# roboyu/Kimera-Multi

Hardware: AMD Instinct MI355X
Metric: dpgo edges*iters/sec (+ LC candidates verified/sec in 'lcd') (higher is better)
Workload: dtype f64

## Files before the change

### kimera-multi_amd/csrc/pgo.hip

```cpp
#include <hip/hip_runtime.h>
#include <hip/hip_ext.h>
#include <rccl/rccl.h>
#include <dlfcn.h>

#include <algorithm>
#include <chrono>
#include <thread>
#include <type_traits>
#include <cmath>
#include <cstdio>
#include <cstdlib>
#include <cstring>
#include <limits>
#include <numeric>
#include <string>
#include <vector>

#include "common.h"

#ifndef KMX_HESS_PROBE
#define KMX_HESS_PROBE 0
#endif

namespace {
// ... 1168 lines not shown
    for (int k = 0; k < j; ++k) s -= Lm[j * 4 + k] * Lm[j * 4 + k];
    Lm[j * 4 + j] = sqrt(s);
    for (int ii = j + 1; ii < 4; ++ii) {
      double t = A[ii * 4 + j];
      for (int k = 0; k < j; ++k) t -= Lm[ii * 4 + k] * Lm[j * 4 + k];
      Lm[ii * 4 + j] = t / Lm[j * 4 + j];
    }
  }
  for (int c = 0; c < 4; ++c)
    for (int ii = 0; ii < 4; ++ii) {
      double s = (ii == c) ? 1.0 : 0.0;
      for (int k = c; k < ii; ++k) s -= Lm[ii * 4 + k] * Li[k * 4 + c];
      Li[ii * 4 + c] = (ii < c) ? 0.0 : s / Lm[ii * 4 + ii];
    }
  double* Pi = d.Pinv + SYM4 * (size_t)pose;
  int j = 0;
  for (int x = 0; x < 4; ++x)
    for (int y = x; y < 4; ++y) {
      double s = 0.0;
      for (int k = 0; k < 4; ++k) s += Li[k * 4 + x] * Li[k * 4 + y];
      Pi[j++] = s;
    }
}

template <int R, int RW, int RM>
__device__ __forceinline__ void body_grad(const Dev& d, int gated, char* smem) {
  const Lane L = lane_map<R>(d);
  if (gated) {
    if (L.tile == 0 && threadIdx.x == 0) store_gnc(d.gnc, load_gnc(d.gnc_next));
    if (d.gnc_next->fired) {
      const int np = L.np, p0 = L.p0;
      for (int t = threadIdx.x; t < np; t += blockDim.x) pose_precond<RW>(d, p0 + t);
      __syncthreads();
    }
  }
  if (d.ctl[L.l].phase != PH_START) return;
  double y[4] = {0, 0, 0, 0}, G[4], cost = 0.0;
  hinc_grad<R, RW>(d, L, d.X, d.pub, G, &cost, smem);
  if (L.valid) load4(d.X + (size_t)L.pose * 4 * R + 4 * L.a, y);
  constexpr int NDP = R >= 5 ? 1 : 2;
  double2 dpart[NDP];
  {
    const double2* Dp2 = reinterpret_cast<const double2*>(d.hD + SYM4 * (size_t)L.pose);
#pragma unroll
    for (int u = 0; u < NDP; ++u) {
      const int i = L.a + u * R;
      dpart[u] = (L.valid && i < 5) ? Dp2[i] : make_double2(0.0, 0.0);
    }
  }
  double S[9], gr[4], zr[4];
  double* scr = reinterpret_cast<double*>(smem);
  group_symYtG<R, true>(y, G, L.base, S, scr);
#pragma unroll
  for (int c = 0; c < 3; ++c) gr[c] = G[c] - (y[0] * S[0 * 3 + c] + y[1] * S[1 * 3 + c] + y[2] * S[2 * 3 + c]);
  gr[3] = G[3];
  group_precon<R, true>(d, L.pose, L.valid, y, gr, L.base, zr, scr);
  double vals[3] = {cost, 0.0, 0.0};
  if (L.valid) {
    vals[1] = gr[0] * gr[0] + gr[1] * gr[1] + gr[2] * gr[2] + gr[3] * gr[3];
    vals[2] = zr[0] * gr[0] + zr[1] * gr[1] + zr[2] * gr[2] + zr[3] * gr[3];
  }
  finish_tile<RED_GRAD, 3, RM>(d, L, vals, smem + SmemHG<R>::red_off, [&]() {
    if (!L.valid) return;
    const size_t o = (size_t)L.pose * 4 * R + 4 * L.a;
    store4(d.g + o, gr);
    store4(d.z + o, zr);
    if (L.a == 0) {
      double* Sp = d.S + 6 * (size_t)L.pose;
      Sp[0] = S[0]; Sp[1] = S[1]; Sp[2] = S[2]; Sp[3] = S[4]; Sp[4] = S[5]; Sp[5] = S[8];
    }
    double2* Fp2 = reinterpret_cast<double2*>(d.hDS + SYM4 * (size_t)L.pose);
#pragma unroll
    for (int u = 0; u < NDP; ++u) {
      const int i = L.a + u * R;
      if (i < 5) {
        const double sx = i == 0 ? S[0] : i == 1 ? S[2] : i == 2 ? S[4] : 0.0;
        const double sy = i == 0 ? S[1] : i == 2 ? S[5] : i == 3 ? S[8] : 0.0;
        Fp2[i] = make_double2(dpart[u].x - sx, dpart[u].y - sy);
      }
    }
  });
}

template <bool LAST>
__device__ __forceinline__ void eta_rows(const Dev& d, int l, size_t o, int T, double clast, double et[4]) {
  const int dhn = d.dhn;
  const int F = T > 0 ? (T - 1) / dhn * dhn : 0;
  if (F > 0) load4(d.eta + o, et);
  double dd[DHMAX][4];
#pragma unroll
  for (int i = 0; i < DHMAX; ++i)
    if (F + i < T) load4(d.dh + (size_t)i * d.vec + o, dd[i]);
  const double* ch = d.coefh + (size_t)l * d.p.tcg_max;
#pragma unroll
  for (int i = 0; i < DHMAX; ++i)
    if (F + i < T) {
      const double cj = (LAST && F + i == T - 1) ? clast : ch[F + i];
#pragma unroll
      for (int k = 0; k < 4; ++k) et[k] += cj * dd[i][k];
    }
}

template <int R>
__device__ __forceinline__ void trial_rows(const Dev& d, const Lane& L, size_t o, const double x[4],
                                           const double gg[4], const double rr[4], const double et[4], char* smem) {
  double xt[4];
  group_retract<R>(x, et, L.base, xt);
  double vals[2] = {0.0, 0.0};
  if (L.valid) {
    store4(d.Xt + o, xt);
    double m = 0.0, ch = 0.0;
#pragma unroll
    for (int k = 0; k < 4; ++k) {
      m += et[k] * (gg[k] + rr[k]);
      const double dd = xt[k] - x[k];
      ch += dd * dd;
    }
    vals[0] = m;
    vals[1] = ch;
  }
  double* lds = reinterpret_cast<double*>(smem);
#pragma unroll
  for (int s = 0; s < 2; ++s) {
    const double w = wave_sum(vals[s]);
    if ((threadIdx.x & 63) == 0) lds[s * WAVES + (threadIdx.x >> 6)] = w;
  }
  __syncthreads();
  if (threadIdx.x == 0) {
#pragma unroll
    for (int s = 0; s < 2; ++s) {
      double t = 0.0;
#pragma unroll
      for (int w = 0; w < WAVES; ++w) t += lds[s * WAVES + w];
      d.part[(size_t)L.tile * NPART + 2 + s] = t;
    }
  }
}

template <int R, int RW, int RM>
struct HessPF {
  static constexpr bool rows = RW == 10 && (R >= 5 || RM == RM_CONSUMER);
};
template <int R, int RW, int RM, bool GRAD, bool EARLY>
__device__ __forceinline__ void body_hess(const Dev& d, int gated, int slot, HostStatus* hs,
                                          unsigned long long seq, char* smem) {
  static_assert(RM == RM_CONSUMER || (!GRAD && !EARLY), "the launched form has one body");
  const Lane L = lane_map<R>(d);
  int tcg_iter;
  double beta;
  double y[4] = {0, 0, 0, 0}, zs[4] = {0, 0, 0, 0}, H[4];
  const size_t o = (size_t)L.pose * 4 * R + 4 * L.a;
  const int dhn = d.dhn;
  double dold[4] = {0, 0, 0, 0}, hold[4] = {0, 0, 0, 0};
  double2 dg[5];
  bool first;
  auto epi = [&]() {
    if (L.valid) {
#if KMX_HESS_PROBE & 2
      for (int k = 0; k < 4; ++k) zs[k] = 1e-3 * k;
      for (int c = 0; c < 5; ++c) dg[c] = make_double2(c == 0 || c == 2 ? 1.0 : 0.0, c >= 3 ? 1.0 : 0.0);
#else
      load4(d.z + o, zs);
      const double2* p2 = reinterpret_cast<const double2*>(d.hDS + SYM4 * (size_t)L.pose);
#pragma unroll
      for (int c = 0; c < 5; ++c) dg[c] = p2[c];
#endif
      if (!first) {
        load4(d.dh + (size_t)((tcg_iter - 1) % dhn) * d.vec + o, dold);
        load4(d.hd + o, hold);
      }
    }
  };
  if constexpr (RM == RM_CONSUMER) {
    __shared__ Ctl cs;
    __shared__ double rl[NPART * WAVES];
    const Ctl& c0 = d.ctl[L.l];
    const bool writer = L.tile == L.rt0;
    if (writer && threadIdx.x < (int)(sizeof(Ctl) / 8))
      reinterpret_cast<double*>(&cs)[threadIdx.x] = reinterpret_cast<const double*>(&c0)[threadIdx.x];
    using RS = std::conditional_t<GRAD, RobotSum<3>, RobotSum<2>>;
    const double* const part = GRAD ? d.part : d.part_u;
    constexpr int stride = GRAD ? NPART : 2;
    RS rs;
// ... 25 lines not shown
      if (writer && threadIdx.x == 0) {
        control_on(cs, d, L.l, GRAD ? RED_GRAD : RED_UPDATE, tot, R, true);
        d.ctl2[L.l] = cs;
        if (hs) post_status(hs, L.l, seq, cs.phase == PH_TCG);
      }
      return !u.done;
    };
    bool go;
    if constexpr (EARLY) {
      go = hinc_gather<R, RW, false, false, HessPF<R, RW, RM>::rows>(d, L, d.z, H, smem, decide, epi);
    } else {
      auto epi_late = [&]() {
        epi();
        rs.issue(part, stride, L.rt0, L.rt1);
      };
      hinc_gather<R, RW, false, false, HessPF<R, RW, RM>::rows>(d, L, d.z, H, smem, NoPre{}, epi_late);
      go = decide();
    }
    if (!go) return;
    beta = u.beta;
  } else {
    const Ctl& c = d.ctl[L.l];
    const int ph = c.phase;
    tcg_iter = c.tcg_iter;
    beta = c.beta;
    first = (tcg_iter == 0) || (KMX_HESS_PROBE & 4);
    if (gated && ph != PH_TCG) return;
    if (!hinc_gather<R, RW, true, false, HessPF<R, RW, RM>::rows>(d, L, d.z, H, smem,
                                                                  [&]() { return ph == PH_TCG; }, epi))
      return;
  }
  if (L.valid) {
    double Dg[16];
    expand_sym4(dg, Dg);
#pragma unroll
    for (int c = 0; c < 4; ++c)
      H[c] += zs[0] * Dg[4 * c] + zs[1] * Dg[4 * c + 1] + zs[2] * Dg[4 * c + 2] + zs[3] * Dg[4 * c + 3];
  }
  double hz[4];
#pragma unroll
  for (int k = 0; k < 4; ++k) hz[k] = H[k];
  (void)y;
  double v = 0.0;
  double dl[4] = {0, 0, 0, 0}, hdl[4] = {0, 0, 0, 0};
  if (L.valid) {
    if (first) {
#pragma unroll
      for (int k = 0; k < 4; ++k) { dl[k] = -zs[k]; hdl[k] = -hz[k]; }
    } else {
#pragma unroll
      for (int k = 0; k < 4; ++k) {
        dl[k] = -zs[k] + beta * dold[k];
        hdl[k] = -hz[k] + beta * hold[k];
      }
      if (tcg_iter >= dhn && tcg_iter % dhn == 0) {
        double et[4] = {0, 0, 0, 0};
        if (tcg_iter > dhn) load4(d.eta + o, et);
        const double* ch = d.coefh + (size_t)L.l * d.p.tcg_max;
        for (int j = tcg_iter - dhn; j < tcg_iter; ++j) {
          double dj[4];
          if (j + 1 < tcg_iter) {
            load4(d.dh + (size_t)(j % dhn) * d.vec + o, dj);
          } else {
#pragma unroll
            for (int k = 0; k < 4; ++k) dj[k] = dold[k];
          }
          const double cj = ch[j];
#pragma unroll
          for (int k = 0; k < 4; ++k) et[k] += cj * dj[k];
        }
        store4(d.eta + o, et);
      }
    }
    v = dl[0] * hdl[0] + dl[1] * hdl[1] + dl[2] * hdl[2] + dl[3] * hdl[3];
  }
  finish_tile<RED_HESS, 1, RM>(d, L, &v, smem + SmemH<R>::red_off, [&]() {
    if (L.valid && !(KMX_HESS_PROBE & 8)) {
      store4(d.dh + (size_t)(tcg_iter % dhn) * d.vec + o, dl);
      store4(d.hd + o, hdl);
    }
  });
}

template <int R, int RM>
__device__ __forceinline__ void body_update(const Dev& d, HostStatus* hs, unsigned long long seq, int slot,
                                            char* smem) {
  const Lane L = lane_map<R>(d);
  int tcg_iter, mode;
  double coef;
  const size_t o = (size_t)L.pose * 4 * R + 4 * L.a;
  double rr[4] = {0, 0, 0, 0}, y[4] = {0, 0, 0, 0}, hdl[4] = {0, 0, 0, 0};
  if constexpr (RM == RM_CONSUMER) {
    __shared__ Ctl cs;
    __shared__ double rl[NPART * WAVES];
    Ctl* const cin = d.ctl2;
    Ctl* const cout = d.ctl;
    const Ctl& cq = cin[L.l];
    const bool writer = L.tile == L.rt0;
    if (writer && threadIdx.x < (int)(sizeof(Ctl) / 8))
      reinterpret_cast<double*>(&cs)[threadIdx.x] = reinterpret_cast<const double*>(&cq)[threadIdx.x];
    if (cq.phase != PH_TCG) {
      if (cq.phase == PH_STEP && !cq.retracted) {
        const size_t o2 = (size_t)L.pose * 4 * R + 4 * L.a;
        double x[4] = {0, 0, 0, 0}, gg[4] = {0, 0, 0, 0}, rr2[4] = {0, 0, 0, 0}, et[4] = {0, 0, 0, 0};
        if (L.valid) {
          load4(d.X + o2, x);
          load4(d.g + o2, gg);
          load4(d.r + o2, rr2);
          eta_rows<false>(d, L.l, o2, cq.tcg_iter, 0.0, et);
        }
        trial_rows<R>(d, L, o2, x, gg, rr2, et, smem);
        if (writer) ctl_publish(cout + L.l, cs, true);
        return;
      }
      if (writer) ctl_publish(cout + L.l, cs, false);
      return;
    }
    const bool first0 = cq.tcg_iter == 0;
    RobotSum<1, 4> rs;
    rs.issue(d.part_h, 2, L.rt0, L.rt1);
    if (L.valid) {
      load4(d.hd + o, hdl);
      load4((first0 ? d.g : d.r) + o, rr);
      load4(d.X + o, y);
    }
    double tot[NPART] = {0.0, 0.0, 0.0, 0.0};
    rs.finish(d.part_h, 2, rl, tot);
    const HessStep hsx = hess_step(cq.z_r, cq.e_Pe, cq.e_Pd, cq.d_Pd, cq.Delta, tot[0]);
    if (writer && threadIdx.x < 64) {
      if (threadIdx.x == 0) {
        control_on(cs, d, L.l, RED_HESS, tot, R, true);
        if (slot >= 0) atomicAdd(d.hv_launch + slot, 1);
      }
      __builtin_amdgcn_wave_barrier();
      asm volatile("" ::: "memory");
      ctl_publish(cout + L.l, cs, false);
    }
    tcg_iter = cq.tcg_iter + 1;
    mode = hsx.boundary ? MODE_BOUNDARY : MODE_INTERIOR;
    coef = hsx.coef;
  } else {
    const Ctl& c = d.ctl[L.l];
    if (c.phase != PH_TCG) {
      if (hs && threadIdx.x == 0 && L.tile == L.rt0) post_status(hs, L.l, seq, false);
      return;
    }
    tcg_iter = c.tcg_iter;
    mode = c.mode;
    coef = c.coef;
    if (L.valid) {
      load4(d.hd + o, hdl);
      load4((tcg_iter == 1 ? d.g : d.r) + o, rr);
      load4(d.X + o, y);
    }
  }
  const bool interior = (mode == MODE_INTERIOR);
  (void)tcg_iter;
  {
    double hp[4];
    group_proj<R, true>(y, hdl, L.base, hp, reinterpret_cast<double*>(smem));
    if (L.valid) {
#pragma unroll
      for (int k = 0; k < 4; ++k) rr[k] += coef * hp[k];
    }
  }
  double vals[2] = {0.0, 0.0}, zr[4] = {0, 0, 0, 0};
  if (interior) {
    group_precon<R, true>(d, L.pose, L.valid, y, rr, L.base, zr, reinterpret_cast<double*>(smem));
    if (L.valid) {
      vals[0] = rr[0] * rr[0] + rr[1] * rr[1] + rr[2] * rr[2] + rr[3] * rr[3];
      vals[1] = zr[0] * rr[0] + zr[1] * rr[1] + zr[2] * rr[2] + zr[3] * rr[3];
    }
  }
  finish_tile<RED_UPDATE, 2, RM>(d, L, vals, smem + SmemU::red_off, [&]() {
    if (L.valid) {
      store4(d.r + o, rr);
      if (interior) store4(d.z + o, zr);
    }
  });
}

__device__ __forceinline__ void onesync_scalars(double al, const double* tot, double* rrn, double* zrn) {
#pragma clang fp contract(off)
  *rrn = fmax(tot[2] + 2.0 * al * tot[5] + al * al * tot[6], 0.0);
  *zrn = tot[1] + al * tot[3] + al * al * tot[4];
}

template <int U>
struct RobotSum8 {
  double a[U][8];
  int t0, t1;
  __device__ __forceinline__ void load(const double* part, int tb) {
#pragma unroll
    for (int u = 0; u < U; ++u) {
      const int t = min(tb + (int)threadIdx.x + u * RBLOCK, t1 - 1);
#pragma unroll
      for (int k = 0; k < 4; ++k) {
        const double2 x = ldpart(part, (size_t)t * 8 + 2 * k);
        a[u][2 * k] = x.x;
        a[u][2 * k + 1] = x.y;
      }
    }
  }
  __device__ __forceinline__ void issue(const double* part, int t0_, int t1_) {
    t0 = t0_;
    t1 = t1_;
    if (t1 - t0 <= U * RBLOCK) load(part, t0);
  }
  __device__ __forceinline__ void finish(const double* part, double* lds, double tot[8]) {
    constexpr int RW_ = RBLOCK / 64;
    double v[8];
#pragma unroll
    for (int k = 0; k < 8; ++k) v[k] = 0.0;
    for (int tb = t0; tb < t1; tb += U * RBLOCK) {
      if (t1 - t0 > U * RBLOCK) load(part, tb);
#pragma unroll
      for (int u = 0; u < U; ++u)
        if (tb + (int)threadIdx.x + u * RBLOCK < t1 && threadIdx.x < RBLOCK) {
#pragma unroll
          for (int k = 0; k < 8; ++k) v[k] += a[u][k];
        }
    }
    __syncthreads();
#pragma unroll
    for (int k = 0; k < 8; ++k) {
      const double w = wave_sum(v[k]);
      if ((threadIdx.x & 63) == 0 && threadIdx.x < RBLOCK) lds[k * RW_ + (threadIdx.x >> 6)] = w;
    }
    __syncthreads();
#pragma unroll
    for (int k = 0; k < 8; ++k) {
      double acc = 0.0;
#pragma unroll
      for (int w = 0; w < RW_; ++w) acc += lds[k * RW_ + w];
      tot[k] = acc;
    }
  }
};

template <int R, int W = WAVES>
struct SmemF {
  static constexpr int red_off = SmemH<R, W>::red_off;
  static constexpr int bytes = red_off + 8 * 8 * W + 16;
};

__device__ __forceinline__ double dot4(const double a[4], const double b[4]) {
  return a[0] * b[0] + a[1] * b[1] + a[2] * b[2] + a[3] * b[3];
}

// ... 191 lines not shown
#pragma unroll
  for (int s2 = 0; s2 < 7; ++s2) {
    const double w = wave_sum(pv[s2]);
    if ((threadIdx.x & 63) == 0) lds[s2 * WAVES + (threadIdx.x >> 6)] = w;
  }
  __syncthreads();
  if (threadIdx.x < 8) {
    double t = 0.0;
    if (threadIdx.x < 7) {
#pragma unroll
      for (int w = 0; w < WAVES; ++w) t += lds[threadIdx.x * WAVES + w];
    }
    d.part_f[((size_t)(kn & 1) * d.ntiles + L.tile) * 8 + threadIdx.x] = t;
  }
  if (L.valid) {
    store4(d.dh + (size_t)(kn % dhn) * d.vec + o, dl);
    store4(d.hd + o, hdl);
    store4(d.hz + o, hzn);
    if (!grad) store4(d.z + o, zn);
    store4(((kn & 1) ? d.w1 : d.w0) + o, wn);
    store4(d.r + o, rn);
  }
#ifdef KMX_STEP_STAMPS
  KMX_SS(6);
  if (kn == 2 && threadIdx.x == 0 && L.tile < STEP_STAMP_TILES) {
    for (int i = 0; i < 7; ++i) g_step_stamp[(size_t)L.tile * 16 + i] = ss_[i];
    g_step_stamp[(size_t)L.tile * 16 + 8] = (unsigned long long)L.np;
    g_step_stamp[(size_t)L.tile * 16 + 9] = (unsigned long long)L.n;
    g_step_stamp[(size_t)L.tile * 16 + 10] = (unsigned long long)blockIdx.x;
    g_step_stamp[(size_t)L.tile * 16 + 11] = (unsigned long long)(L.tile == L.rt0);
  }
#endif
}

template <int R>
__device__ __forceinline__ void body_retract(const Dev& d, int fold, const Ctl* src, char* smem) {
  const Lane L = lane_map<R>(d);
  const Ctl& c = src[L.l];
  __shared__ int sph;
  __shared__ double rl[NPART * WAVES];
  if (threadIdx.x == 0) {
    sph = c.phase;
    if (src != d.ctl && L.tile == L.rt0) d.ctl[L.l] = c;
  }
  __syncthreads();
  const int ph = sph;
  const size_t o = (size_t)L.pose * 4 * R + 4 * L.a;
  double x[4] = {0, 0, 0, 0}, et[4] = {0, 0, 0, 0}, gg[4] = {0, 0, 0, 0}, rr[4] = {0, 0, 0, 0}, dl[4];
  if (fold && ph == PH_TCG) {
    RobotSum<2> rs;
    rs.issue(d.part_u, 2, L.rt0, L.rt1);
    double tot[NPART] = {0.0, 0.0, 0.0, 0.0};
    rs.finish(d.part_u, 2, rl, tot);
    const UpdStep u = upd_step(c.mode, c.r_stop, c.lin_stop, c.z_r, c.tcg_iter, tot[0], tot[1], d.p);
    if (!u.done) return;
    if (threadIdx.x == 0 && L.tile == L.rt0) {
      if (u.stop >= 0) d.ctl[L.l].tcg_stop = u.stop;
      d.ctl[L.l].phase = PH_STEP;
    }
  } else if (ph != PH_STEP || (fold == 2 && c.retracted)) {
    return;
  }
  if (L.valid) {
    load4(d.X + o, x);
    load4(d.g + o, gg);
    load4(d.r + o, rr);
    if (d.p.rgd) {
      load4(d.z + o, dl);
      const double coef = c.coef;
#pragma unroll
      for (int k = 0; k < 4; ++k) et[k] += coef * dl[k];
    } else {
      eta_rows<false>(d, L.l, o, c.tcg_iter, 0.0, et);
    }
  }
  trial_rows<R>(d, L, o, x, gg, rr, et, smem);
}

template <int R, int RW, int RM>
__device__ __forceinline__ void body_cost(const Dev& d, const Ctl* src, char* smem) {
  const Lane L = lane_map<R>(d);
  const Ctl& c = src[L.l];
  if (src != d.ctl && threadIdx.x == 0 && L.tile == L.rt0) d.ctl[L.l] = c;
  if (c.phase != PH_STEP) return;
  double cost = inc_owner_cost<R, RW>(d, L, d.Xt, d.pub, smem);
  finish_tile<RED_COST, 1, RM>(d, L, &cost, smem + SmemC<R>::red_off, []() {});
}

template <int R>
__device__ __forceinline__ void body_commit(const Dev& d, int fold, int final) {
  const Lane L = lane_map<R>(d);
  if (final && L.tile == 0 && threadIdx.x == 0) {
    d.gnc->inner += 1;
    d.gnc->rounds += 1;
  }
  bool commit;
  if (fold) {
    __shared__ int sph;
    __shared__ Ctl cs;
    __shared__ double rl[NPART * WAVES];
    const Ctl& c = d.ctl[L.l];
    const bool writer = L.tile == L.rt0;
    if (writer && threadIdx.x < (int)(sizeof(Ctl) / 8))
      reinterpret_cast<double*>(&cs)[threadIdx.x] = reinterpret_cast<const double*>(&c)[threadIdx.x];
    if (threadIdx.x == 0) sph = c.phase;
    __syncthreads();
    if (sph != PH_STEP) return;
    RobotSum<NPART> rs;
    rs.issue(d.part, NPART, L.rt0, L.rt1);
    double tot[NPART] = {0.0, 0.0, 0.0, 0.0};
    rs.finish(d.part, NPART, rl, tot);
    if (d.p.rgd) {
      commit = true;
    } else {
      const double model_dec = -0.5 * tot[2];
      const double rho = (model_dec > 0.0) ? (c.f_cur - tot[0]) / model_dec : -1.0;
      commit = rho > d.p.accept_rho;
    }
    if (threadIdx.x == 0 && writer) {
      control_on(cs, d, L.l, RED_COST, tot, R, true);
      cs.phase = PH_STEP;
      d.ctl[L.l] = cs;
    }
  } else {
    commit = d.ctl[L.l].commit != 0;
  }
  if (!commit || !L.valid) return;
  const size_t o = (size_t)L.pose * 4 * R + 4 * L.a;
  double v[4];
  load4(d.Xt + o, v);
  store4(d.X + o, v);
  if (!final) return;
  const int s = d.pose_slot[L.pose];
  if (s >= 0) store4(d.pub + (size_t)s * 4 * R + 4 * L.a, v);
}

template <int R, int RW, int RM>
__global__ __launch_bounds__(BLOCK, LB<R>::w) void k_grad(Dev d, int gated) {
  KMX_SMEM;
  body_grad<R, RW, RM>(d, gated, smem);
}
template <int R, int RW, int RM, bool GRAD, bool EARLY>
__global__ __launch_bounds__(BLOCK, LB<R>::w) void k_hess(Dev d, int gated, int slot, HostStatus* hs,
                                                          unsigned long long seq) {
  KMX_SMEM;
  body_hess<R, RW, RM, GRAD, EARLY>(d, gated, slot, hs, seq, smem);
}
template <int R, int RM>
__global__ __launch_bounds__(BLOCK) void k_update(Dev d, HostStatus* hs, unsigned long long seq, int slot) {
  KMX_SMEM;
  body_update<R, RM>(d, hs, seq, slot, smem);
}
template <int R, int RW>
__global__ __launch_bounds__(BLOCK, (R <= 5 ? 3 : 2)) void k_step(Dev d, const Ctl* cin, Ctl* cout, int jl, int slot,
                                                                  HostStatus* hs, unsigned long long seq) {
  KMX_SMEM;
  body_step<R, RW>(d, cin, cout, jl, slot, hs, seq, smem);
}
template <int R>
__global__ __launch_bounds__(BLOCK) void k_retract(Dev d, int fold, const Ctl* src) {
  KMX_SMEM;
  body_retract<R>(d, fold, src, smem);
}
template <int R, int RW, int RM>
__global__ __launch_bounds__(BLOCK, LB<R>::w) void k_cost(Dev d, const Ctl* src) {
  KMX_SMEM;
  body_cost<R, RW, RM>(d, src, smem);
}
template <int R>
__global__ __launch_bounds__(BLOCK) void k_commit(Dev d, int fold, int final) {
  body_commit<R>(d, fold, final);
}

__device__ __forceinline__ bool gnc_should_update(const Dev& d) {
  const Params& P = d.p;
  if (!P.robust || !P.gnc_on) return false;
  const Gnc& s = *d.gnc;
  if (s.updates >= P.max_updates) return false;
  if (s.inner > P.inner_iters) return true;
  for (int l = 0; l < d.L; ++l)
    if (!(d.relc[l] <= P.rel_tol)) return false;
  for (int k = 0; k < P.n_ext; ++k)
    if (!(d.ext[k] <= P.rel_tol)) return false;
  return true;
}

template <int RW>
__device__ __forceinline__ void gnc_edge(const Dev& d, int i, int R_, double mu) {
  const int e = d.gnc_edge[i];
  const int2 en = d.gnc_ends[i];
  const int ps = 4 * R_;
  const double* Xi = en.x >= 0 ? d.X + (size_t)en.x * ps : d.pub + (size_t)(-1 - en.x) * ps;
  const double* Xj = en.y >= 0 ? d.X + (size_t)en.y * ps : d.pub + (size_t)(-1 - en.y) * ps;
  const int2 ip = d.eipos[e];
  double2 q[Rec<RW>::Q];
  Rec<RW>::load(d, (size_t)(ip.x >= 0 ? ip.x : ip.y), q);
  Edge E;
  Rec<RW>::edge(q, E);
  double sR = 0.0, sT = 0.0;
  for (int a = 0; a < R_; ++a) {
    const double* yi = Xi + 4 * a;
    const double* yj = Xj + 4 * a;
    for (int c = 0; c < 3; ++c) {
      const double r = yj[c] - (yi[0] * E.R[0 * 3 + c] + yi[1] * E.R[1 * 3 + c] + yi[2] * E.R[2 * 3 + c]);
      sR += r * r;
    }
    const double et = yj[3] - yi[3] - (yi[0] * E.t[0] + yi[1] * E.t[1] + yi[2] * E.t[2]);
    sT += et * et;
  }
  const double rSq = d.ekappa[e] * sR + d.etau[e] * sT;
  const double barcSq = d.p.barc * d.p.barc;
  const double upper = (mu + 1.0) / mu * barcSq;
  const double lower = mu / (mu + 1.0) * barcSq;
  double w;
  if (rSq >= upper) w = 0.0;
  else if (rSq <= lower) w = 1.0;
  else w = sqrt(barcSq * mu * (mu + 1.0) / rSq) - mu;
  d.ew[e] = w;
  const double wk = w * d.ekappa[e], wt = w * d.etau[e];
  constexpr int WK = Rec<RW>::WK;
  constexpr int GS = Rec<RW>::GS;
  if (ip.x >= 0) { d.rec[(size_t)GS * ip.x + WK] = wk; d.rec[(size_t)GS * ip.x + WK + 1] = Rec<RW>::wt_word(wt, true); }
  if (ip.y >= 0) { d.rec[(size_t)GS * ip.y + WK] = wk; d.rec[(size_t)GS * ip.y + WK + 1] = Rec<RW>::wt_word(wt, false); }
}

__device__ __forceinline__ void begin_robot(const Dev& d, const unsigned char* active, int l) {
  Ctl& c = d.ctl[l];
  const bool a = active ? active[l] != 0 : true;
  const Ctl zero = {};
  c = zero;
  c.phase = a ? PH_START : PH_IDLE;
  c.updated = a ? 1 : 0;
  c.Delta = d.p.Delta0;
}

enum BeginMode { BEGIN_ROUND = 1, BEGIN_FORCE_GNC = 2, BEGIN_SOLO = 4 };

template <int RW>
__global__ void k_begin(Dev d, const unsigned char* active, int mode, int R_) {
  const bool fire = d.p.robust && ((mode & BEGIN_FORCE_GNC) ? true : gnc_should_update(d));
  const double mu = d.gnc->mu;
  if (blockIdx.x == 0) {
    if (mode & BEGIN_ROUND)
      for (int l = threadIdx.x; l < d.L; l += blockDim.x) begin_robot(d, active, l);
    if (threadIdx.x == 0) {
      Gnc s = load_gnc(d.gnc);
      s.fired = fire ? 1 : 0;
      if (fire) {
        s.inner = 0;
        s.updates += 1;
        s.mu = mu * d.p.mu_step;
      }
      store_gnc(d.gnc_next, s);
      if (mode & BEGIN_SOLO) store_gnc(d.gnc, s);
// ... 307 lines not shown
  bool own_stream = false;
  int n_robots = 0;
  std::vector<int> npose;
  std::vector<int> local_of;
  std::vector<int> robots;
  std::vector<int> loff;
  int nloc = 0;
  int64_t m_global = 0;
  int64_t npub = 0, first_owned = 0, n_owned = 0;
  std::vector<int64_t> pub_key;
  int mloc = 0;
  std::vector<int64_t> loc_edge_gid;
  int ninc = 0;
  int rw = 10;
  int64_t nshared = 0;
  int n_sh_local = 0, n_gnc = 0, n_osh = 0;
  std::vector<long long> m_robot;
  int ntiles = 0;
  std::vector<int> rt0_h;
  int gnc_on = 0, gnc_inner_iters = 20, gnc_max_updates = 0x7fffffff, n_ext = 0;
  double gnc_rel_tol = 1e-3;
  Dev dv{};
  TileDesc* d_tile = nullptr;
  int* d_rtile0 = nullptr;
  int* d_inc_ptr = nullptr;
  double* d_rec = nullptr;
  int* d_rec_o = nullptr;
  double *d_ekappa = nullptr, *d_etau = nullptr, *d_ew = nullptr;
  int2* d_eipos = nullptr;
  double* d_vec = nullptr;
  double* d_coefh = nullptr;
  double* d_part_f = nullptr;
  int ctl_par = 0;
  double *d_S = nullptr, *d_Pinv = nullptr, *d_hD = nullptr, *d_hDS = nullptr, *d_pub = nullptr, *d_part = nullptr;
  Ctl* d_ctl = nullptr;
  Ctl* d_ctl2 = nullptr;
  double *d_part_h = nullptr, *d_part_u = nullptr;
  Counters* d_cnt = nullptr;
  long long* d_m_robot = nullptr;
  int* d_n_robot = nullptr;
  int* d_pub_src = nullptr;
  int* d_own_src = nullptr;
  int* d_pose_slot = nullptr;
  int* d_gnc_edge = nullptr;
  int2* d_gnc_ends = nullptr;
  int *d_sh_edge = nullptr, *d_sh_idx = nullptr;
  int *d_osh_edge = nullptr, *d_osh_idx = nullptr;
  double* d_relc = nullptr;
  Gnc* d_gnc = nullptr;
  double* d_ext = nullptr;
  int ext_cap = 0;
  unsigned char* d_active = nullptr;
  double* d_scratch = nullptr;
  size_t scratch_cap = 0;
  HostStatus* hstat = nullptr;
  int hstat_cap = 0;
  unsigned long long seq = 0;
  bool poll = true;
  bool poll_auto = true;
  ncclComm_t comm = nullptr;
  int world = 1, rank = 0;
  bool xchg = false, xchg_self_p2p = false;
  int *d_xs_slots = nullptr, *d_xr_slots = nullptr, *d_xs_seg = nullptr, *d_xr_seg = nullptr;
  int *d_xs_rseg = nullptr, *d_xr_rseg = nullptr;
  double *d_xsbuf = nullptr, *d_xrbuf = nullptr;
  long long xn_send = 0, xn_recv = 0;
  std::vector<long long> xs_cnt, xr_cnt, xs_off, xr_off;
  static constexpr int BLIND_SLACK = 2, BLIND_WINDOW = 8;
  static constexpr int MAX_GROUPS = 4;
  struct Group {
    int l0 = 0, l1 = 0;
    int t0 = 0, nt = 0;
    int blind_left = 0;
  };
  int groups_req = 2;
  std::vector<Group> grp;
  Group all;
  int grm = 2;
  int grm_forced = -1;
  static constexpr int GROUP_CONSUMER_MAX_TILES = 384;
  hipStream_t gstream[MAX_GROUPS - 1] = {nullptr, nullptr, nullptr};
  hipEvent_t ev_fork = nullptr, ev_join[MAX_GROUPS - 1] = {nullptr, nullptr, nullptr};
  bool hess_gate = true;
  int rm = RM_LAUNCH;
  int rm_forced = -1;
  int early_stop = 1;
  int decide_forced = -1;
  static constexpr int RM_CONSUMER_MAX_POSES = 80000;
  bool poll_timeout = false;
  bool timing = false;
  int* d_hv_launch = nullptr;
  std::vector<hipEvent_t> ev_pool;
  size_t ev_used = 0;
  double *d_accV = nullptr, *d_accY = nullptr;
  double acc_gamma = 0.0;
  int acc_k = 0;
  bool acc_ready = false, acc_started = false;
};

namespace {

void rot_to_quat(const double* R, double* q) {
  const double tr = R[0] + R[4] + R[8];
  double w, x, y, z;
  if (tr > 0.0) {
    const double s = 2.0 * std::sqrt(tr + 1.0);
    w = 0.25 * s; x = (R[7] - R[5]) / s; y = (R[2] - R[6]) / s; z = (R[3] - R[1]) / s;
  } else if (R[0] > R[4] && R[0] > R[8]) {
    const double s = 2.0 * std::sqrt(1.0 + R[0] - R[4] - R[8]);
    w = (R[7] - R[5]) / s; x = 0.25 * s; y = (R[1] + R[3]) / s; z = (R[2] + R[6]) / s;
  } else if (R[4] > R[8]) {
    const double s = 2.0 * std::sqrt(1.0 + R[4] - R[0] - R[8]);
    w = (R[2] - R[6]) / s; x = (R[1] + R[3]) / s; y = 0.25 * s; z = (R[5] + R[7]) / s;
  } else {
    const double s = 2.0 * std::sqrt(1.0 + R[8] - R[0] - R[4]);
    w = (R[3] - R[1]) / s; x = (R[2] + R[6]) / s; y = (R[5] + R[7]) / s; z = 0.25 * s;
  }
  const double n = std::sqrt(w * w + x * x + y * y + z * z);
  q[0] = w / n; q[1] = x / n; q[2] = y / n; q[3] = z / n;
}
int quat_pack(const double* q, double* q3) {
  int big = 0;
  for (int i = 1; i < 4; ++i)
    if (std::fabs(q[i]) > std::fabs(q[big])) big = i;
  const double sg = q[big] < 0.0 ? -1.0 : 1.0;
  for (int i = 0, j = 0; i < 4; ++i)
    if (i != big) q3[j++] = sg * q[i];
  return big;
}
void quat_unpack(const double* q3, int big, double* q) {
  const double ql = std::sqrt(1.0 - (q3[0] * q3[0] + q3[1] * q3[1] + q3[2] * q3[2]));
  for (int i = 0, j = 0; i < 4; ++i) q[i] = i == big ? ql : q3[j++];
}
void quat_to_rot(const double* q, double* R) {
  const double w = q[0], x = q[1], y = q[2], z = q[3];
  const double xx = x * x, yy = y * y, zz = z * z, xy = x * y, xz = x * z, yz = y * z;
  const double wx = w * x, wy = w * y, wz = w * z;
  R[0] = 1.0 - 2.0 * (yy + zz); R[1] = 2.0 * (xy - wz); R[2] = 2.0 * (xz + wy);
  R[3] = 2.0 * (xy + wz); R[4] = 1.0 - 2.0 * (xx + zz); R[5] = 2.0 * (yz - wx);
  R[6] = 2.0 * (xz - wy); R[7] = 2.0 * (yz + wx); R[8] = 1.0 - 2.0 * (xx + yy);
}

template <typename T>
int dalloc(T** p, size_t count) {
  *p = nullptr;
  if (count == 0) count = 1;
  hipError_t e = hipMalloc(reinterpret_cast<void**>(p), sizeof(T) * count);
  if (e != hipSuccess) return kmx::fail(KMX_ENOMEM, std::string("hipMalloc: ") + hipGetErrorString(e));
  return 0;
}

template <typename... T>
void free_all(T*&... p) {
  (((p ? (void)hipFree(p) : (void)0), p = nullptr), ...);
}

void free_xchg(kmx_pgo* h) {
  free_all(h->d_xs_slots, h->d_xr_slots, h->d_xs_seg, h->d_xr_seg, h->d_xs_rseg, h->d_xr_rseg, h->d_xsbuf,
           h->d_xrbuf);
  h->xchg = false;
}

void free_dev(kmx_pgo* h) {
  free_all(h->d_tile, h->d_rtile0, h->d_inc_ptr, h->d_rec, h->d_rec_o, h->d_ekappa, h->d_etau, h->d_ew, h->d_eipos,
           h->d_vec, h->d_S, h->d_Pinv, h->d_hD, h->d_hDS, h->d_pub, h->d_part, h->d_ctl, h->d_cnt, h->d_m_robot,
           h->d_n_robot, h->d_pub_src, h->d_own_src, h->d_pose_slot, h->d_gnc_edge, h->d_gnc_ends, h->d_sh_edge,
// ... 110 lines not shown

bool wait_running(kmx_pgo* h, unsigned long long seq, int l0, int l1) {
  volatile HostStatus* hs = h->hstat;
  const auto t0 = std::chrono::steady_clock::now();
  bool running = false;
  for (int l = l0; l < l1; ++l) {
    if (h->rt0_h[l + 1] == h->rt0_h[l]) continue;
    unsigned long long w;
    while (((w = __atomic_load_n(&hs[l].word, __ATOMIC_ACQUIRE)) >> 1) < seq) {
      if (std::chrono::steady_clock::now() - t0 > std::chrono::seconds(30)) {
        h->poll_timeout = true;
        h->poll = false;
        return true;
      }
    }
    running |= (w & 1ull) != 0;
  }
  return running;
}

int groups_in_effect(const kmx_pgo* h) {
  if (h->timing || h->rm != RM_LAUNCH || h->P.method != KMX_METHOD_RTR || onesync(h)) return 1;
  return std::max<int>(1, (int)h->grp.size());
}

struct Chain {
  Dev d;
  hipStream_t s;
  int l0, nl;
  kmx_pgo::Group* st;
};
Chain make_chain(kmx_pgo* h, kmx_pgo::Group& G, hipStream_t s) {
  Chain q{h->dv, s, G.l0, G.l1 - G.l0, &G};
  q.d.gt0 = G.t0;
  q.d.gnt = G.nt;
  return q;
}
template <int R>
void red(const Chain& q, int kind, HostStatus* hs = nullptr, unsigned long long seq = 0, int slot = -1,
         hipEvent_t done = nullptr) {
  if (done)
    hipExtLaunchKernelGGL(k_reduce, dim3(q.nl), dim3(RBLOCK), 0, q.s, nullptr, done, 0u, q.d, q.l0, kind, R, hs, seq,
                          slot, (const double*)nullptr);
  else
    hipLaunchKernelGGL(k_reduce, dim3(q.nl), dim3(RBLOCK), 0, q.s, q.d, q.l0, kind, R, hs, seq, slot,
                       (const double*)nullptr);
}

struct Timed {
  int slot = -1;
  hipEvent_t e0 = nullptr, e1 = nullptr;
};
Timed next_timed(kmx_pgo* h) {
  Timed t;
  if (h->timing && h->ev_used / 2 < (size_t)HV_SLOTS) {
    t.slot = (int)(h->ev_used / 2);
    t.e0 = next_event(h);
    t.e1 = next_event(h);
  }
  return t;
}

bool tcg_polls(kmx_pgo* h, kmx_pgo::Group& st) {
  if (!(h->poll && h->hstat)) return false;
  if (h->poll_auto && st.blind_left > 0) {
    --st.blind_left;
    return false;
  }
  return true;
}
void tcg_polled(const kmx_pgo* h, kmx_pgo::Group& st, bool poll, int steps) {
  if (poll && h->poll_auto && steps + kmx_pgo::BLIND_SLACK >= h->P.tcg_max_iterations)
    st.blind_left = kmx_pgo::BLIND_WINDOW;
}

template <int RM>
bool fold_grad(const kmx_pgo* h) {
  return RM == RM_CONSUMER && h->P.method != KMX_METHOD_RGD && h->P.tcg_max_iterations > 0;
}
template <int RM>
bool fold_cost(const kmx_pgo* h) {
  return RM == RM_CONSUMER && (h->P.rtr_iterations == 1 || h->P.method == KMX_METHOD_RGD);
}

template <int R, int RW, int RM>
void launch_hess(const kmx_pgo* h, dim3 grid, hipStream_t st, const Dev& dv, int fl, int slot, HostStatus* hs,
                 unsigned long long seq, hipEvent_t e0 = nullptr, hipEvent_t e1 = nullptr) {
  const dim3 blk(BLOCK);
  const int gated = (fl & 2) ? 1 : 0;
  auto go = [&](auto kern) {
    if (e0)
      hipExtLaunchKernelGGL(kern, grid, blk, SmemH<R>::bytes, st, e0, e1, 0u, dv, gated, slot, hs, seq);
    else
      hipLaunchKernelGGL(kern, grid, blk, SmemH<R>::bytes, st, dv, gated, slot, hs, seq);
  };
  if constexpr (RM == RM_CONSUMER) {
    const bool grad = (fl & 1) != 0, early = h->early_stop != 0;
    if (grad && early) go(k_hess<R, RW, RM, true, true>);
    else if (grad) go(k_hess<R, RW, RM, true, false>);
    else if (early) go(k_hess<R, RW, RM, false, true>);
    else go(k_hess<R, RW, RM, false, false>);
  } else {
    go(k_hess<R, RW, RM, false, false>);
  }
}

template <int R, int RW, int RM>
void enqueue_tcg_t(kmx_pgo* h, const Chain* q, int G, bool* stopped) {
  constexpr bool cons = RM == RM_CONSUMER;
  const dim3 blk(BLOCK);
  const int tmax = h->P.tcg_max_iterations;
  bool poll[kmx_pgo::MAX_GROUPS], live[kmx_pgo::MAX_GROUPS];
  unsigned long long prev[kmx_pgo::MAX_GROUPS], seq[kmx_pgo::MAX_GROUPS];
  int steps[kmx_pgo::MAX_GROUPS];
  for (int g = 0; g < G; ++g) {
    poll[g] = tcg_polls(h, *q[g].st);
    live[g] = true;
    prev[g] = seq[g] = 0;
    steps[g] = tmax;
  }
  for (int j = 0; j < tmax; ++j) {
    bool any = false;
    for (int g = 0; g < G; ++g) {
      if (!live[g]) continue;
      any = true;
      const Timed t = next_timed(h);
      poll[g] = poll[g] && h->poll;
      seq[g] = poll[g] ? ++h->seq : 0;
      HostStatus* hs = poll[g] ? h->hstat : nullptr;
      const int fl = (j == 0 ? 1 : 0) | (j > 0 && h->hess_gate ? 2 : 0);
      const dim3 grid(q[g].d.gnt);
      if constexpr (cons) {
        launch_hess<R, RW, RM>(h, grid, q[g].s, q[g].d, fl, t.slot, hs, seq[g], t.e0, t.e1);
        hipLaunchKernelGGL((k_update<R, RM>), grid, blk, SmemU::bytes, q[g].s, q[g].d, (HostStatus*)nullptr, 0ull,
                           t.slot);
      } else {
        launch_hess<R, RW, RM>(h, grid, q[g].s, q[g].d, fl, t.slot, nullptr, 0ull, t.e0, t.e1);
        red<R>(q[g], RED_HESS, nullptr, 0, t.slot);
        hipLaunchKernelGGL((k_update<R, RM>), grid, blk, SmemU::bytes, q[g].s, q[g].d, (HostStatus*)nullptr, seq[g],
                           -1);
        red<R>(q[g], RED_UPDATE, hs, seq[g]);
      }
    }
    if (!any) break;
    for (int g = 0; g < G; ++g) {
      if (!live[g] || !poll[g]) continue;
      if (j > 0 && !wait_running(h, cons ? seq[g] : prev[g], q[g].l0, q[g].l0 + q[g].nl)) {
        steps[g] = j + 1;
        live[g] = false;
        stopped[g] = true;
      }
      prev[g] = seq[g];
    }
  }
  for (int g = 0; g < G; ++g) tcg_polled(h, *q[g].st, poll[g], steps[g]);
}

template <int R, int RW>
void enqueue_tcg_onesync_t(kmx_pgo* h, const Chain& q) {
  const dim3 grid(q.d.gnt), blk(BLOCK);
  const int tmax = h->P.tcg_max_iterations;
  bool poll = tcg_polls(h, *q.st);
  int J = tmax + 1;
  for (int j = 0; j <= tmax; ++j) {
    const Timed t = next_timed(h);
    poll = poll && h->poll;
    const unsigned long long seq = poll ? ++h->seq : 0;
    HostStatus* hs = poll ? h->hstat : nullptr;
    const Ctl* cin = (j & 1) ? h->d_ctl2 : h->d_ctl;
    Ctl* cout = (j & 1) ? h->d_ctl : h->d_ctl2;
    if (t.e0)
      hipExtLaunchKernelGGL((k_step<R, RW>), grid, blk, SmemF<R>::bytes, q.s, t.e0, t.e1, 0u, q.d, cin, cout, j,
                            t.slot, hs, seq);
    else
      hipLaunchKernelGGL((k_step<R, RW>), grid, blk, SmemF<R>::bytes, q.s, q.d, cin, cout, j, t.slot, hs, seq);
    if (poll && j > 0 && !wait_running(h, seq, q.l0, q.l0 + q.nl)) {
      J = j + 1;
      break;
    }
  }
  h->ctl_par = J & 1;
  tcg_polled(h, *q.st, poll, J - 1);
}

template <int R, int RW, int RM>
void enqueue_round_t(kmx_pgo* h, const unsigned char* d_active, int G) {
  constexpr bool cons = RM == RM_CONSUMER;
  const dim3 blk(BLOCK);
  const bool rgd = h->P.method == KMX_METHOD_RGD, os = cons && onesync(h);
  const bool pend = enqueue_begin(h, d_active, BEGIN_ROUND, true, G > 1 ? h->ev_fork : nullptr);
  Chain q[kmx_pgo::MAX_GROUPS];
  if (G == 1) q[0] = make_chain(h, h->all, h->stream);
  else
    for (int g = 0; g < G; ++g) q[g] = make_chain(h, h->grp[g], g == 0 ? h->stream : h->gstream[g - 1]);
  for (int g = 1; g < G; ++g) (void)hipStreamWaitEvent(q[g].s, h->ev_fork, 0);
  const int iters = rgd ? 1 : h->P.rtr_iterations;
  const bool fgrad = fold_grad<RM>(h), fcost = fold_cost<RM>(h);
  for (int it = 0; it < iters; ++it) {
    for (int g = 0; g < G; ++g) {
      hipLaunchKernelGGL((k_grad<R, RW, RM>), dim3(q[g].d.gnt), blk, SmemHG<R>::bytes, q[g].s, q[g].d,
                         it == 0 && pend ? 1 : 0);
      if (!fgrad) red<R>(q[g], RED_GRAD);
    }
    bool stopped[kmx_pgo::MAX_GROUPS] = {};
    if constexpr (cons) {
      if (os) enqueue_tcg_onesync_t<R, RW>(h, q[0]);
    }
    if (!rgd && !os) enqueue_tcg_t<R, RW, RM>(h, q, G, stopped);
    const Ctl* src = os && h->ctl_par ? h->d_ctl2 : h->d_ctl;
    for (int g = 0; g < G; ++g) {
      const dim3 grid(q[g].d.gnt);
      const bool last = it + 1 == iters;
      hipEvent_t join = g > 0 && last ? h->ev_join[g - 1] : nullptr;
      if (!os && !(cons && stopped[g]))
        hipLaunchKernelGGL((k_retract<R>), grid, blk, SmemU::bytes, q[g].s, q[g].d, cons && !rgd ? 2 : 0,
                           (const Ctl*)h->d_ctl);
      if (fcost && join)
        hipExtLaunchKernelGGL((k_cost<R, RW, RM>), grid, blk, SmemC<R>::bytes, q[g].s, nullptr, join, 0u, q[g].d, src);
      else
        hipLaunchKernelGGL((k_cost<R, RW, RM>), grid, blk, SmemC<R>::bytes, q[g].s, q[g].d, src);
      if (!fcost) red<R>(q[g], RED_COST, nullptr, 0, -1, join);
      if (!last)
        hipLaunchKernelGGL((k_commit<R>), grid, blk, 0, q[g].s, q[g].d, 0, 0);
    }
  }
  for (int g = 1; g < G; ++g) (void)hipStreamWaitEvent(h->stream, h->ev_join[g - 1], 0);
  hipLaunchKernelGGL((k_commit<R>), dim3(h->ntiles), blk, 0, h->stream, h->dv, fcost ? 1 : 0, 1);
}

void enqueue_round(kmx_pgo* h, const unsigned char* d_active) {
  const int G = groups_in_effect(h);
  const int rm = G > 1 ? h->grm : h->rm;
  with_r(h->P.r, [&](auto R) {
    constexpr int r = decltype(R)::value;
    if (rm == RM_CONSUMER)
      with_rw(h->rw, [&](auto RW) { enqueue_round_t<r, RW(), RM_CONSUMER>(h, d_active, G); });
    else
      with_rw(h->rw, [&](auto RW) { enqueue_round_t<r, RW(), RM_LAUNCH>(h, d_active, G); });
  });
}

double accel_gamma_next(const kmx_pgo* h) {
  const double N = (double)h->n_robots;
  return (1.0 + std::sqrt(1.0 + 4.0 * N * N * h->acc_gamma * h->acc_gamma)) / (2.0 * N);
}
void launch_accel(kmx_pgo* h, double c, int mode) {
  with_r(h->P.r, [&](auto R) {
    hipLaunchKernelGGL(k_accel<R()>, dim3(h->ntiles), dim3(BLOCK), 0, h->stream, h->dv, h->d_accV, h->d_accY, c, mode);
  });
}
void enqueue_accel_pre(kmx_pgo* h) {
  if (!h->P.acceleration || h->acc_ready || h->ntiles == 0) return;
  if (!h->acc_started) {
    launch_accel(h, 0.0, 2);
    h->acc_started = true;
  }
  const double g = accel_gamma_next(h);
  launch_accel(h, 1.0 / (g * (double)h->n_robots), 0);
  h->acc_ready = true;
}
void enqueue_accel_post(kmx_pgo* h) {
  if (!h->P.acceleration || !h->acc_ready || h->ntiles == 0) return;
  const double g = accel_gamma_next(h);
  const bool restart = h->P.restart_interval > 0 && (h->acc_k + 1) % h->P.restart_interval == 0;
  launch_accel(h, g, restart ? 2 : 1);
  h->acc_gamma = restart ? 0.0 : g;
  h->acc_k = restart ? 0 : h->acc_k + 1;
  h->acc_ready = false;
}
void accel_reset(kmx_pgo* h) {
  h->acc_gamma = 0.0;
  h->acc_k = 0;
  h->acc_ready = h->acc_started = false;
}

void enqueue_apply_weights(kmx_pgo* h) {
  if (h->mloc > 0)
    with_rw(h->rw, [&](auto RW) {
      hipLaunchKernelGGL(k_apply_weights<RW()>, dim3((h->mloc + 255) / 256), dim3(256), 0, h->stream, h->dv, h->mloc);
    });
  enqueue_precond(h, 0);
}

}

extern "C" int kmx_pgo_create(const kmx_pgo_params* params, int device, kmx_pgo** out) {
  KMX_GUARD_BEGIN
  KMX_CHECK(params && out, KMX_EINVAL, "null argument");
  KMX_CHECK(params->d == 3, KMX_EUNSUP, "only d = 3 is supported");
  KMX_CHECK(params->r >= 3 && params->r <= 8, KMX_EUNSUP, "relaxation rank must be in [3, 8]");
  KMX_CHECK(params->rtr_iterations >= 1 && params->tcg_max_iterations >= 1, KMX_EINVAL,
            "rtr_iterations and tcg_max_iterations must be >= 1");
  KMX_CHECK(params->robust_cost == KMX_COST_L2 || params->robust_cost == KMX_COST_GNC_TLS, KMX_EUNSUP,
            "robust cost must be L2 or GNC_TLS");
  KMX_CHECK((params->acceleration == 0 || params->acceleration == 1) && params->restart_interval >= 0, KMX_EINVAL,
            "acceleration is 0 or 1, restart_interval >= 0");
  KMX_CHECK(params->method == KMX_METHOD_RTR || params->method == KMX_METHOD_RGD, KMX_EUNSUP,
            "method must be KMX_METHOD_RTR or KMX_METHOD_RGD");
  KMX_CHECK(params->tcg_form == KMX_TCG_FORM_STANDARD || params->tcg_form == KMX_TCG_FORM_ONESYNC, KMX_EINVAL,
            "tcg_form must be KMX_TCG_FORM_STANDARD or KMX_TCG_FORM_ONESYNC");
  KMX_CHECK(params->method != KMX_METHOD_RGD || params->rgd_stepsize > 0.0, KMX_EINVAL, "rgd_stepsize must be > 0");
  KMX_CHECK(params->tile_incidences >= 0, KMX_EINVAL, "tile_incidences must be >= 0 (0: automatic)");
  int ndev = 0;
  KMX_HIP(hipGetDeviceCount(&ndev));
  KMX_CHECK(device >= 0 && device < ndev, KMX_EINVAL, "bad HIP device ordinal");
  KMX_HIP(hipSetDevice(device));
  kmx_pgo* h = new kmx_pgo();
  h->P = *params;
  h->device = device;
  hipError_t e = hipStreamCreateWithFlags(&h->stream, hipStreamNonBlocking);
  if (e != hipSuccess) {
    delete h;
    return kmx::fail(KMX_EHIP, std::string("hipStreamCreate: ") + hipGetErrorString(e));
  }
  h->own_stream = true;
  if (const char* v = std::getenv("KMX_RED")) {
    const int m = std::atoi(v);
    h->rm_forced = m == 0 ? RM_LAUNCH : m == 2 ? RM_CONSUMER : -1;
  }
  if (const char* v = std::getenv("KMX_HESS_DECIDE")) h->decide_forced = std::atoi(v) != 0 ? 1 : 0;
  if (const char* v = std::getenv("KMX_HESS_GATE")) h->hess_gate = std::atoi(v) != 0;
  if (const char* v = std::getenv("KMX_TCG_GROUPS")) {
    const int g = std::atoi(v);
    h->groups_req = g >= 4 ? 4 : g >= 2 ? 2 : 1;
  }
  if (const char* v = std::getenv("KMX_GROUP_RED")) h->grm_forced = std::atoi(v) == 2 ? RM_CONSUMER : RM_LAUNCH;
  for (int g = 1; g < h->groups_req && e == hipSuccess; ++g) {
    e = hipStreamCreateWithFlags(&h->gstream[g - 1], hipStreamNonBlocking);
    if (e == hipSuccess) e = hipEventCreate(&h->ev_join[g - 1]);
  }
  if (e == hipSuccess && h->groups_req > 1) e = hipEventCreate(&h->ev_fork);
  if (e != hipSuccess) {
    (void)kmx_pgo_destroy(h);
    return kmx::fail(KMX_EHIP, std::string("robot group streams: ") + hipGetErrorString(e));
  }
  *out = h;
  return KMX_OK;
  KMX_GUARD_END
}

extern "C" int kmx_pgo_destroy(kmx_pgo* h) {
  if (!h) return KMX_OK;
  (void)hipSetDevice(h->device);
  if (h->stream) (void)hipStreamSynchronize(h->stream);
  for (hipStream_t s : h->gstream)
    if (s) (void)hipStreamSynchronize(s);
  free_dev(h);
  free_xchg(h);
  if (h->comm) (void)ncclCommAbort(h->comm);
  for (auto e : h->ev_pool) (void)hipEventDestroy(e);
  if (h->own_stream && h->stream) (void)hipStreamDestroy(h->stream);
  if (h->hstat) (void)hipHostFree(h->hstat);
  for (hipStream_t s : h->gstream)
    if (s) (void)hipStreamDestroy(s);
  for (hipEvent_t ev : h->ev_join)
    if (ev) (void)hipEventDestroy(ev);
  if (h->ev_fork) (void)hipEventDestroy(h->ev_fork);
  delete h;
  return KMX_OK;
}

extern "C" int kmx_pgo_set_stream(kmx_pgo* h, void* s) {
  KMX_CHECK(h, KMX_EINVAL, "null handle");
  KMX_HIP(hipSetDevice(h->device));
  if (h->own_stream && h->stream) {
    KMX_HIP(hipStreamSynchronize(h->stream));
    KMX_HIP(hipStreamDestroy(h->stream));
  }
  h->own_stream = false;
  h->stream = reinterpret_cast<hipStream_t>(s);
  return KMX_OK;
}

extern "C" int kmx_pgo_set_tcg_poll(kmx_pgo* h, int mode) {
  KMX_CHECK(h, KMX_EINVAL, "null handle");
  KMX_CHECK(mode >= -1 && mode <= 1, KMX_EINVAL, "mode is -1 (adaptive), 0 (blind) or 1 (polled)");
  h->poll = mode != 0;
  h->poll_auto = mode == -1;
  h->all.blind_left = 0;
  for (auto& g : h->grp) g.blind_left = 0;
  return KMX_OK;
}

extern "C" int kmx_pgo_get_tcg_groups(kmx_pgo* h, int* groups, int32_t* bounds) {
  KMX_CHECK(h && groups, KMX_EINVAL, "null argument");
  *groups = ready(h) ? groups_in_effect(h) : 1;
  if (bounds) {
    const int G = ready(h) ? (int)h->grp.size() : 0;
    for (int g = 0; g <= kmx_pgo::MAX_GROUPS; ++g)
      bounds[g] = g < G ? h->grp[g].l0 : G > 0 ? h->grp[G - 1].l1 : 0;
  }
  return KMX_OK;
}

extern "C" int kmx_pgo_get_group_reduction(kmx_pgo* h, int* form) {
  KMX_CHECK(h && form, KMX_EINVAL, "null argument");
  *form = ready(h) && groups_in_effect(h) > 1 ? h->grm : h->rm;
  return KMX_OK;
}

extern "C" int kmx_pgo_set_graph(kmx_pgo* h, int n_robots, const int32_t* n_poses, const uint8_t* local,
                                 int64_t m, const int32_t* r1, const int32_t* p1, const int32_t* r2,
                                 const int32_t* p2, const double* R, const double* t, const double* kappa,
                                 const double* tau, const double* weight, const uint8_t* fixed_weight) {
// ... 1116 lines not shown
```

Before: 1.033 billion.

## Fuse last tCG update with retraction and fold update decision into cost kernel

Adds a k_update_last variant for the final truncated-CG iteration in consumer-reduction mode. It computes the residual update, accumulates eta from the stored direction history and writes the trial retraction in the same kernel. The separate k_retract launch is dropped when this tail path is enabled. The cost kernel now also handles robots still in the TCG phase whose step was retracted: it finishes the update reduction and moves them to the step phase. This saves one launch per RTR iteration and reuses already-loaded vectors, but it skips preconditioning on the last iteration and adds more control-state branching.

New measurement: 1.055 billion, median of 6. +2.1%, better.

```diff
diff --git a/kimera-multi_amd/csrc/pgo.hip b/kimera-multi_amd/csrc/pgo.hip
--- a/kimera-multi_amd/csrc/pgo.hip
+++ b/kimera-multi_amd/csrc/pgo.hip
@@ -1274,23 +1274,34 @@
   });
 }
 
+struct EtaRows {
+  double dd[DHMAX][4];
+  int F;
+  __device__ __forceinline__ void issue(const Dev& d, size_t o, int T, double et[4]) {
+    const int dhn = d.dhn;
+    F = T > 0 ? (T - 1) / dhn * dhn : 0;
+    if (F > 0) load4(d.eta + o, et);
+#pragma unroll
+    for (int i = 0; i < DHMAX; ++i)
+      if (F + i < T) load4(d.dh + (size_t)i * d.vec + o, dd[i]);
+  }
+  template <bool LAST>
+  __device__ __forceinline__ void finish(const Dev& d, int l, int T, double clast, double et[4]) const {
+    const double* ch = d.coefh + (size_t)l * d.p.tcg_max;
+#pragma unroll
+    for (int i = 0; i < DHMAX; ++i)
+      if (F + i < T) {
+        const double cj = (LAST && F + i == T - 1) ? clast : ch[F + i];
+#pragma unroll
+        for (int k = 0; k < 4; ++k) et[k] += cj * dd[i][k];
+      }
+  }
+};
 template <bool LAST>
 __device__ __forceinline__ void eta_rows(const Dev& d, int l, size_t o, int T, double clast, double et[4]) {
-  const int dhn = d.dhn;
-  const int F = T > 0 ? (T - 1) / dhn * dhn : 0;
-  if (F > 0) load4(d.eta + o, et);
-  double dd[DHMAX][4];
-#pragma unroll
-  for (int i = 0; i < DHMAX; ++i)
-    if (F + i < T) load4(d.dh + (size_t)i * d.vec + o, dd[i]);
-  const double* ch = d.coefh + (size_t)l * d.p.tcg_max;
-#pragma unroll
-  for (int i = 0; i < DHMAX; ++i)
-    if (F + i < T) {
-      const double cj = (LAST && F + i == T - 1) ? clast : ch[F + i];
-#pragma unroll
-      for (int k = 0; k < 4; ++k) et[k] += cj * dd[i][k];
-    }
+  EtaRows e;
+  e.issue(d, o, T, et);
+  e.finish<LAST>(d, l, T, clast, et);
 }
 
 template <int R>
@@ -1482,14 +1493,18 @@
   });
 }
 
-template <int R, int RM>
+template <int R, int RM, bool LAST = false>
 __device__ __forceinline__ void body_update(const Dev& d, HostStatus* hs, unsigned long long seq, int slot,
                                             char* smem) {
+  static_assert(!LAST || RM == RM_CONSUMER, "the launched form keeps k_retract");
   const Lane L = lane_map<R>(d);
   int tcg_iter, mode;
   double coef;
   const size_t o = (size_t)L.pose * 4 * R + 4 * L.a;
   double rr[4] = {0, 0, 0, 0}, y[4] = {0, 0, 0, 0}, hdl[4] = {0, 0, 0, 0};
+  double gg[4] = {0, 0, 0, 0}, et[4] = {0, 0, 0, 0};
+  EtaRows er;
+  int T = 0;
   if constexpr (RM == RM_CONSUMER) {
     __shared__ Ctl cs;
     __shared__ double rl[NPART * WAVES];
@@ -1517,12 +1532,23 @@
       return;
     }
     const bool first0 = cq.tcg_iter == 0;
+    if constexpr (LAST) {
+      T = cq.tcg_iter + 1;
+      if (T != d.p.tcg_max) {
+        if (writer) ctl_publish(cout + L.l, cs, false);
+        return;
+      }
+    }
     RobotSum<1, 4> rs;
     rs.issue(d.part_h, 2, L.rt0, L.rt1);
     if (L.valid) {
       load4(d.hd + o, hdl);
       load4((first0 ? d.g : d.r) + o, rr);
       load4(d.X + o, y);
+      if constexpr (LAST) {
+        load4(d.g + o, gg);
+        er.issue(d, o, T, et);
+      }
     }
     double tot[NPART] = {0.0, 0.0, 0.0, 0.0};
     rs.finish(d.part_h, 2, rl, tot);
@@ -1534,7 +1560,7 @@
       }
       __builtin_amdgcn_wave_barrier();
       asm volatile("" ::: "memory");
-      ctl_publish(cout + L.l, cs, false);
+      ctl_publish(cout + L.l, cs, LAST);
     }
     tcg_iter = cq.tcg_iter + 1;
     mode = hsx.boundary ? MODE_BOUNDARY : MODE_INTERIOR;
@@ -1565,6 +1591,15 @@
     }
   }
   double vals[2] = {0.0, 0.0}, zr[4] = {0, 0, 0, 0};
+  if constexpr (LAST) {
+    if (interior && L.valid) vals[0] = rr[0] * rr[0] + rr[1] * rr[1] + rr[2] * rr[2] + rr[3] * rr[3];
+    finish_tile<RED_UPDATE, 2, RM>(d, L, vals, smem + SmemU::red_off, [&]() {
+      if (L.valid) store4(d.r + o, rr);
+    });
+    if (L.valid) er.template finish<true>(d, L.l, T, coef, et);
+    trial_rows<R>(d, L, o, y, gg, rr, et, smem);
+    return;
+  }
   if (interior) {
     group_precon<R, true>(d, L.pose, L.valid, y, rr, L.base, zr, reinterpret_cast<double*>(smem));
     if (L.valid) {
@@ -1922,9 +1957,28 @@
   const Lane L = lane_map<R>(d);
   const Ctl& c = src[L.l];
   if (src != d.ctl && threadIdx.x == 0 && L.tile == L.rt0) d.ctl[L.l] = c;
-  if (c.phase != PH_STEP) return;
+  const int ph = c.phase;
+  bool go = ph == PH_STEP;
+  if constexpr (RM == RM_CONSUMER) {
+    go = go || (ph == PH_TCG && c.retracted);
+  }
+  if (!go) return;
   double cost = inc_owner_cost<R, RW>(d, L, d.Xt, d.pub, smem);
   finish_tile<RED_COST, 1, RM>(d, L, &cost, smem + SmemC<R>::red_off, []() {});
+  if constexpr (RM == RM_CONSUMER) {
+    if (L.tile == L.rt0 && c.phase == PH_TCG) {
+      __shared__ double rl[NPART * WAVES];
+      RobotSum<2> rs;
+      rs.issue(d.part_u, 2, L.rt0, L.rt1);
+      double tot[NPART] = {0.0, 0.0, 0.0, 0.0};
+      rs.finish(d.part_u, 2, rl, tot);
+      const UpdStep u = upd_step(c.mode, c.r_stop, c.lin_stop, c.z_r, c.tcg_iter, tot[0], tot[1], d.p);
+      if (threadIdx.x == 0) {
+        if (u.stop >= 0) d.ctl[L.l].tcg_stop = u.stop;
+        d.ctl[L.l].phase = PH_STEP;
+      }
+    }
+  }
 }
 
 template <int R>
@@ -2010,6 +2064,11 @@
 template <int R>
 __global__ __launch_bounds__(BLOCK) void k_commit(Dev d, int fold, int final) {
   body_commit<R>(d, fold, final);
+}
+template <int R>
+__global__ __launch_bounds__(BLOCK) void k_update_last(Dev d, HostStatus* hs, unsigned long long seq, int slot) {
+  KMX_SMEM;
+  body_update<R, RM_CONSUMER, true>(d, hs, seq, slot, smem);
 }
 
 __device__ __forceinline__ bool gnc_should_update(const Dev& d) {
@@ -2483,6 +2542,7 @@
   hipStream_t gstream[MAX_GROUPS - 1] = {nullptr, nullptr, nullptr};
   hipEvent_t ev_fork = nullptr, ev_join[MAX_GROUPS - 1] = {nullptr, nullptr, nullptr};
   bool hess_gate = true;
+  bool tcg_tail = true;
   int rm = RM_LAUNCH;
   int rm_forced = -1;
   int early_stop = 1;
@@ -2759,6 +2819,11 @@
 bool fold_cost(const kmx_pgo* h) {
   return RM == RM_CONSUMER && (h->P.rtr_iterations == 1 || h->P.method == KMX_METHOD_RGD);
 }
+template <int RM>
+bool tail_fused(const kmx_pgo* h) {
+  return RM == RM_CONSUMER && h->tcg_tail && h->P.method != KMX_METHOD_RGD && !onesync(h) &&
+         h->P.tcg_max_iterations > 0;
+}
 
 template <int R, int RW, int RM>
 void launch_hess(const kmx_pgo* h, dim3 grid, hipStream_t st, const Dev& dv, int fl, int slot, HostStatus* hs,
@@ -2809,8 +2874,12 @@
       const dim3 grid(q[g].d.gnt);
       if constexpr (cons) {
         launch_hess<R, RW, RM>(h, grid, q[g].s, q[g].d, fl, t.slot, hs, seq[g], t.e0, t.e1);
-        hipLaunchKernelGGL((k_update<R, RM>), grid, blk, SmemU::bytes, q[g].s, q[g].d, (HostStatus*)nullptr, 0ull,
-                           t.slot);
+        if (j == tmax - 1 && tail_fused<RM>(h))
+          hipLaunchKernelGGL((k_update_last<R>), grid, blk, SmemU::bytes, q[g].s, q[g].d, (HostStatus*)nullptr, 0ull,
+                             t.slot);
+        else
+          hipLaunchKernelGGL((k_update<R, RM>), grid, blk, SmemU::bytes, q[g].s, q[g].d, (HostStatus*)nullptr, 0ull,
+                             t.slot);
       } else {
         launch_hess<R, RW, RM>(h, grid, q[g].s, q[g].d, fl, t.slot, nullptr, 0ull, t.e0, t.e1);
         red<R>(q[g], RED_HESS, nullptr, 0, t.slot);
@@ -2889,7 +2958,7 @@
       const dim3 grid(q[g].d.gnt);
       const bool last = it + 1 == iters;
       hipEvent_t join = g > 0 && last ? h->ev_join[g - 1] : nullptr;
-      if (!os && !(cons && stopped[g]))
+      if (!os && !(cons && stopped[g]) && !tail_fused<RM>(h))
         hipLaunchKernelGGL((k_retract<R>), grid, blk, SmemU::bytes, q[g].s, q[g].d, cons && !rgd ? 2 : 0,
                            (const Ctl*)h->d_ctl);
       if (fcost && join)
@@ -2997,6 +3066,7 @@
   }
   if (const char* v = std::getenv("KMX_HESS_DECIDE")) h->decide_forced = std::atoi(v) != 0 ? 1 : 0;
   if (const char* v = std::getenv("KMX_HESS_GATE")) h->hess_gate = std::atoi(v) != 0;
+  if (const char* v = std::getenv("KMX_TCG_TAIL")) h->tcg_tail = std::atoi(v) != 0;
   if (const char* v = std::getenv("KMX_TCG_GROUPS")) {
     const int g = std::atoi(v);
     h->groups_req = g >= 4 ? 4 : g >= 2 ? 2 : 1;
```
